# bgmanuel99/Super-Resolution-Images-for-3D-Printing-Defect-Detection

Hardware: AMD Instinct MI355X
Metric: 4x-SR MPix/s on 512x512 LR batch (higher is better)
Workload: dtype bf16

## Files before the change

super-resolution-images-for-3d-printing-defect-detection_amd/csrc/dense_fused.hip:

```cpp
#include <stdlib.h>
#include <string.h>

#include <type_traits>

#include "conv_common.h"

namespace {

struct ChainParams {
    const char* in; int in_nch;
    char* out; int out_nch;
    const char* so; int so_nch;
    const char* w;
    const float* bias;
    const char* zero;
    int B, H;
    int rows_per_wg; unsigned magic;
    float alpha, xscale, oscale;
    int dbg_flags;
    unsigned long long* dbg;
};

__device__ __forceinline__ f32x4 mma16(bf16x8 a, bf16x8 b, f32x4 c) { return __builtin_amdgcn_mfma_f32_16x16x32_bf16(a, b, c, 0, 0, 0); }

constexpr int ROWB = 3072;
constexpr int NSTG = 11;
constexpr int STGB = NSTG * ROWB;
constexpr int WINR = 10;
constexpr int ZERO_PAGE_BYTES = sr_ctx::ZERO_PAGE_BYTES;

template <int NB0, int NB1, int MODE> struct ChainLds {
    static constexpr int WSLOT = (NB0 + NB1) * 3 * 1024;
    static constexpr int NSB = MODE == 0 ? 3 : 2;
    static constexpr int NWS = MODE == 0 ? 2 : 3;
    static constexpr int BYTES = NSB * STGB + WINR * ROWB + NWS * WSLOT + (NB0 + NB1) * 16 * 4;
};

typedef unsigned u32x2 __attribute__((ext_vector_type(2)));
typedef unsigned u32x4 __attribute__((ext_vector_type(4)));
#define CHAIN_STAMP(k) do { if (STAMP && blockIdx.x < 64 && G < 64 && (wave == 0 || wave == 5 || wave == 8 || wave == 11) && lane == 0)                \
        p.dbg[(((size_t)blockIdx.x * 4 + (wave == 0 ? 0 : wave == 5 ? 1 : wave == 8 ? 2 : 3)) * 64 + G) * 4 + (k)] = __builtin_amdgcn_s_memtime(); } while (0)

template <int N, class F> __device__ __forceinline__ void static_for(F&& f) {
    if constexpr (N > 0) {
        static_for<N - 1>(f);
        f(std::integral_constant<int, N - 1>{});
    }
}

template <int N> __device__ __forceinline__ void wait_imm() {
    static_assert(N >= 0 && N < 64, "vmcnt is a 6-bit counter");
    asm volatile("s_waitcnt vmcnt(%0)" ::"n"(N) : "memory");
}

template <int EXT, int NB0, int NB1, int MODE, int LW> struct LoaderPlan {
    static constexpr int NBT = NB0 + NB1, EXTG = 3 * EXT, NGR = 3 * (EXT + 1);
    static constexpr int RT_E = MODE == 1 ? 2 : 3;
    static constexpr int RT_R = 2;
    static constexpr int nrows(int kx) { return kx == 0 ? 2 : kx == 1 ? (LW < 3 ? 1 : 0) : 0; }
    static constexpr int nst_at(int i) {
        i = (i % NGR + NGR) % NGR;
        return i < EXTG ? 3 * nrows(i % 3) : 0;
    }
    static constexpr int nwdma(int iw) {
        const bool ext = iw < EXTG;
        const int nw = ext ? NBT * 3 : NB1 * 3, rt = ext ? RT_E : RT_R;
        int n = 0;
        for (int t = 0; t < (nw + 3) / 4; ++t)
            if (LW + 4 * t < nw && t >= rt) ++n;
        return n;
    }
};

constexpr bool kDirectStores = true;
constexpr int NCOMP = 8, NLOAD = 4;

template <int EXT, int NB0, int NB1, int MODE, bool HAS_O, bool STAMP, bool SEAM = false>
__global__ void __launch_bounds__((NCOMP + NLOAD) * 64, (NCOMP + NLOAD + 3) / 4) chain2_kernel(ChainParams p) {
    using L = ChainLds<NB0, NB1, MODE>;
    constexpr int NBT = NB0 + NB1, WSLOT = L::WSLOT;
    constexpr int NGR = 3 * (EXT + 1);
    constexpr int EXTG = 3 * EXT;
    constexpr int NTHR = (NCOMP + NLOAD) * 64;
    extern __shared__ __attribute__((aligned(16))) char smem[];
    char* const stg = smem;
    constexpr int NSB = L::NSB;
    char* const win = smem + NSB * STGB;
    char* const wr = win + WINR * ROWB;
    constexpr int NWS = L::NWS;
    float* const lbias = reinterpret_cast<float*>(wr + NWS * WSLOT);

    const int tid = threadIdx.x, lane = tid & 63, px = lane & 15, q = lane >> 4;
    const int wave = __builtin_amdgcn_readfirstlane(tid >> 6);
    const int H = p.H, Hp1 = H + 1;
    const int T = p.B * Hp1;
    const int R0 = blockIdx.x * p.rows_per_wg, R1 = min(T, R0 + p.rows_per_wg);
    if (R0 >= R1) return;
    const int Rs = R0 - 1;
    const int N = R1 - Rs + 1;
    const int nsteps = (N + 1 + 7) >> 3;

    for (int u = tid; u < WINR * ROWB / 16; u += NTHR) *reinterpret_cast<f32x4*>(win + u * 16) = f32x4{0.f, 0.f, 0.f, 0.f};
    if (tid < NBT * 16) lbias[tid] = p.bias[tid];
    asm volatile("s_waitcnt lgkmcnt(0)" ::: "memory");
    __builtin_amdgcn_s_barrier();

    auto row_of = [&](int g, int& img, int& y) -> bool {
        const int gg = Rs + g;
        if (gg < 0 || gg >= T) return false;
        img = (int)__umulhi((unsigned)gg, p.magic);
        y = gg - img * Hp1;
        return y < H;
    };
    auto own = [&](int g) { return Rs + g >= R0 && Rs + g < R1; };
    int G = 0;
    auto dma = [&](const char* src, char* dst) {
        __builtin_amdgcn_global_load_lds((const __attribute__((address_space(1))) void*)src, (__attribute__((address_space(3))) void*)dst, 16, 0, 0);
    };
    if (wave >= NCOMP) {
        const int lwr = wave - NCOMP;
        const int lsrc = 64 * (lane >> 2) + 16 * ((lane & 3) ^ (2 * ((lane >> 4) & 1)));
        auto loader = [&](auto LWc) {
            constexpr int LW = decltype(LWc)::value;
            auto row_base = [&](int s2, int j) -> const char* {
                int img, y;
                const bool real = row_of(8 * s2 - 2 + j, img, y);
                return real ? p.in + ((int64_t)img * H + y) * p.in_nch * ROWB : p.zero;
            };
            using Plan = LoaderPlan<EXT, NB0, NB1, MODE, LW>;
            const char* rb_cur[3];
            const char* rb_nxt[3];
            auto bases_of = [&](int s2, const char* (&rb)[3]) {
                rb[0] = row_base(s2, LW);
                rb[1] = row_base(s2, LW + 4);
                rb[2] = row_base(s2, 8 + (LW < 3 ? LW : 2));
            };
            auto stage_row = [&](auto Jc, const char* rb, int c1, char* sdst) {
                constexpr int j = decltype(Jc)::value;
                const char* src = rb + c1 * ROWB + lsrc;
                char* dst = sdst + j * ROWB;
                const auto gs = (const __attribute__((address_space(1))) void*)src;
                const auto ld = (__attribute__((address_space(3))) void*)dst;
                if constexpr (j < 8) {
                    __builtin_amdgcn_global_load_lds(gs, ld, 16, 0, 2);
                    __builtin_amdgcn_global_load_lds(gs, ld, 16, 1024, 2);
                    __builtin_amdgcn_global_load_lds(gs, ld, 16, 2048, 2);
                } else {
                    __builtin_amdgcn_global_load_lds(gs, ld, 16, 0, 0);
                    __builtin_amdgcn_global_load_lds(gs, ld, 16, 1024, 0);
                    __builtin_amdgcn_global_load_lds(gs, ld, 16, 2048, 0);
                }
            };
            auto stage_rows = [&](auto KXc, const char* (&rb)[3], int c1, char* sdst) {
                constexpr int kx = decltype(KXc)::value;
                if constexpr (kx == 0) {
                    stage_row(std::integral_constant<int, LW>{}, rb[0], c1, sdst);
                    stage_row(std::integral_constant<int, LW + 4>{}, rb[1], c1, sdst);
                } else if constexpr (kx == 1 && LW < 3) {
                    stage_row(std::integral_constant<int, 8 + (LW < 3 ? LW : 0)>{}, rb[2], c1, sdst);
                }
            };
            constexpr int RT_E = Plan::RT_E, RT_R = Plan::RT_R;
            u32x4 wre[EXTG][RT_E], wrr[3][RT_R];
            auto wsrc_of = [&](int iw) { return p.w + (iw < EXTG ? iw * WSLOT : EXTG * WSLOT + (iw - EXTG) * (NB1 * 3 * 1024)); };
#pragma unroll
            for (int iw = 0; iw < EXTG; ++iw)
#pragma unroll
                for (int t = 0; t < RT_E; ++t)
                    if (LW + 4 * t < NBT * 3) wre[iw][t] = *reinterpret_cast<const u32x4*>(wsrc_of(iw) + (LW + 4 * t) * 1024 + lane * 16);
#pragma unroll
            for (int r = 0; r < 3; ++r)
#pragma unroll
                for (int t = 0; t < RT_R; ++t)
                    if (LW + 4 * t < NB1 * 3) wrr[r][t] = *reinterpret_cast<const u32x4*>(wsrc_of(EXTG + r) + (LW + 4 * t) * 1024 + lane * 16);
            auto put_weights = [&](auto IW, int Gw) {
                constexpr int iw = decltype(IW)::value;
                constexpr bool ext = iw < EXTG;
                constexpr int nw = ext ? NBT * 3 : NB1 * 3, rt = ext ? RT_E : RT_R;
                const char* wq = p.w;
                asm volatile("" : "+s"(wq));
                const char* wsrc = wq + (ext ? iw * WSLOT : EXTG * WSLOT + (iw - EXTG) * (NB1 * 3 * 1024)) + lane * 16;
                char* wdst = wr + (Gw % NWS) * WSLOT;
#pragma unroll
                for (int t = 0; t < (nw + 3) / 4; ++t) {
                    const int k = LW + 4 * t;
                    if (k < nw) {
                        if (t < rt) {
                            if constexpr (ext) *reinterpret_cast<u32x4*>(wdst + k * 1024 + lane * 16) = wre[ext ? iw : 0][t < RT_E ? t : 0];
                            else *reinterpret_cast<u32x4*>(wdst + k * 1024 + lane * 16) = wrr[ext ? 0 : iw - EXTG][t < RT_R ? t : 0];
                        } else {
                            dma(wsrc + k * 1024, wdst + k * 1024);
                        }
                    }
                }
            };
            constexpr int WL = NWS - 1;
            constexpr int SL = NSB - 1;
            static_assert(MODE == 1 || (RT_E * NLOAD >= NBT * 3 && RT_R * NLOAD >= NB1 * 3), "growth pairs: every weight piece is resident (no weight DMA in the counted waits)");
            static_assert(SL <= EXT, "rows run at most one step ahead");
            static_for<WL>([&](auto I) { put_weights(I, decltype(I)::value); });
            bases_of(0, rb_cur);
            bases_of(1, rb_nxt);
            static_for<SL>([&](auto C0) {
                constexpr int c0 = decltype(C0)::value;
                stage_rows(std::integral_constant<int, 0>{}, rb_cur, c0, stg + c0 * STGB);
                stage_rows(std::integral_constant<int, 1>{}, rb_cur, c0, stg + c0 * STGB);
            });
            int nch = 0;
            for (int s = 0; s < nsteps; ++s) {
                static_for<NGR>([&](auto I) {
                    constexpr int i = decltype(I)::value;
                    CHAIN_STAMP(0);
                    if (G == 0) asm volatile("s_waitcnt vmcnt(0)" ::: "memory");
                    asm volatile("s_waitcnt lgkmcnt(0)" ::: "memory");
                    __builtin_amdgcn_s_barrier();
                    CHAIN_STAMP(1);
                    constexpr int i2 = (i + WL) % NGR;
                    put_weights(std::integral_constant<int, i2>{}, G + WL);
                    if constexpr (i < EXTG) {
                        constexpr int c = i / 3, kx = i - 3 * c;
                        constexpr int c1 = (c + SL) % EXT;
                        constexpr bool next_step = c + SL >= EXT;
                        char* sdst = stg + ((nch + SL) % NSB) * STGB;
                        stage_rows(std::integral_constant<int, kx>{}, next_step ? rb_nxt : rb_cur, c1, sdst);
                        if (kx == 2) ++nch;
                    }
                    CHAIN_STAMP(2);
                    if constexpr (MODE == 0) {
                        wait_imm<Plan::nst_at(i) + Plan::nst_at(i - 1) + Plan::nst_at(i - 2)>();
                    } else {
                        constexpr bool third = i < EXTG && i % 3 == 2;
                        wait_imm<Plan::nwdma(i2) + Plan::nst_at(i) + (third ? 0 : Plan::nst_at(i - 1))>();
                    }
                    CHAIN_STAMP(3);
                    ++G;
                });
                rb_cur[0] = rb_nxt[0]; rb_cur[1] = rb_nxt[1]; rb_cur[2] = rb_nxt[2];
                bases_of(s + 2, rb_nxt);
            }
            asm volatile("s_waitcnt vmcnt(0)" ::: "memory");
        };
        if (lwr == 0) loader(std::integral_constant<int, 0>{});
        else if (lwr == 1) loader(std::integral_constant<int, 1>{});
        else if (lwr == 2) loader(std::integral_constant<int, 2>{});
        else loader(std::integral_constant<int, 3>{});
        return;
    }

    int offk[3];
#pragma unroll
    for (int kx = 0; kx < 3; ++kx) {
        const int c = px + kx - 1;
        offk[kx] = 64 * c + 16 * (q ^ (2 * ((c >> 2) & 1)));
    }
    const bool edge_l = px == 0, edge_r = px == 15;
    const int off_l = edge_l ? offk[1] : offk[0];
    const int off_r = edge_r ? offk[1] : offk[2];
    const bool seam_l = SEAM && px == 8, seam_r = SEAM && px == 7;

    f32x4 a0[NB0][3], a1[NB1][3];

    auto transpose_offsets = [&](int& t_a, int& t_line) {
        int l = lane;
        asm volatile("" : "+v"(l));
        const int px_ = l & 15, q_ = l >> 4;
        t_a = px_ * 64 + 16 * ((q_ >> 1) ^ ((px_ >> 1) & 3)) + (q_ & 1) * 8;
        t_line = (l >> 2) * 64 + 16 * ((l & 3) ^ ((l >> 3) & 3));
    };

    auto xfold = [&](int h, float scale) {
        const bf16_t xs_b = (bf16_t)scale;
        int j0 = 16 * h + px - 8 * q;
        asm volatile("" : "+v"(j0));
        bf16x8 f;
#pragma unroll
        for (int j = 0; j < 8; ++j) f[j] = j == j0 ? xs_b : (bf16_t)0.f;
        return f;
    };
    constexpr int WDEPTH = 3, NWREG = WDEPTH + 1;
    struct ExtStage { int d, layer, n, frag, first; };
    auto ext_stage = [](int k) constexpr -> ExtStage {
        int i = 0;
        for (int d = 0; d < 4; ++d) {
            bool first = true;
            if (d >= 1)
                for (int n = 0; n < NB0; ++n, ++i, first = false)
                    if (i == k) return ExtStage{d, 0, n, (d - 1) * NB0 + n, first};
            if (d <= 2)
                for (int n = 0; n < NB1; ++n, ++i, first = false)
                    if (i == k) return ExtStage{d, 1, n, 3 * NB0 + d * NB1 + n, first};
        }
        return ExtStage{-1, 0, 0, 0, 0};
    };
    constexpr int NEXTST = 3 * (NB0 + NB1);
    auto ext_granule = [&](auto KXc, auto FOLDc, const char* sb, const char* ws) {
        constexpr int KX = decltype(KXc)::value;
        constexpr int FOLD = KX == 1 ? decltype(FOLDc)::value : -1;
        const char* rb = sb + wave * ROWB;
        auto load_row = [&](int d, bf16x8 (&x)[3]) {
#pragma unroll
            for (int cg = 0; cg < 3; ++cg) {
                const int off = (KX == 0 && cg == 0) ? off_l : (KX == 2 && cg == 2) ? off_r : offk[KX];
                x[cg] = *reinterpret_cast<const bf16x8*>(rb + d * ROWB + cg * 1024 + off);
                if ((KX == 0 && cg == 0 && edge_l) || (KX == 2 && cg == 2 && edge_r)) x[cg] = bf16x8{};
                if (SEAM && cg == 1 && ((KX == 0 && seam_l) || (KX == 2 && seam_r))) x[cg] = bf16x8{};
            }
        };
        auto ldw = [&](int frag) { return *reinterpret_cast<const bf16x8*>(ws + frag * 1024 + lane * 16); };
        bf16x8 xr[2][3], wq[NWREG];
        load_row(0, xr[0]);
        static_for<WDEPTH>([&](auto K) { wq[decltype(K)::value] = ldw(ext_stage(decltype(K)::value).frag); });
        static_for<NEXTST>([&](auto K) {
            constexpr int k = decltype(K)::value;
            constexpr ExtStage st = ext_stage(k);
            if constexpr (st.first && st.d < 3) load_row(st.d + 1, xr[(st.d + 1) & 1]);
            if constexpr (k + WDEPTH < NEXTST) wq[(k + WDEPTH) % NWREG] = ldw(ext_stage(k + WDEPTH).frag);
#pragma unroll
            for (int cg = 0; cg < 3; ++cg) {
                if constexpr (st.layer == 0) a0[st.n][cg] = mma16(wq[k % NWREG], xr[st.d & 1][cg], a0[st.n][cg]);
                else a1[st.n][cg] = mma16(wq[k % NWREG], xr[st.d & 1][cg], a1[st.n][cg]);
            }
            if constexpr (FOLD >= 0 && st.d == 1 && st.layer == 1 && st.n == NB1 - 1) {
#pragma unroll
                for (int h = 0; h < 2; ++h) {
                    const bf16x8 f = xfold(h, p.xscale);
#pragma unroll
                    for (int cg = 0; cg < 3; ++cg) a1[2 * FOLD + h][cg] = mma16(f, xr[1][cg], a1[2 * FOLD + h][cg]);
                }
            }
            __builtin_amdgcn_sched_barrier(0);
        });
    };
    constexpr int NRINGST = 3 * NB1;
    auto ring_granule = [&](auto KXc, int s, const char* ws) {
        constexpr int KX = decltype(KXc)::value;
        auto load_row = [&](int ky, bf16x8 (&x)[3]) {
            const char* rb = win + ((8 * s + wave - 2 + ky + 2 * WINR) % WINR) * ROWB;
#pragma unroll
            for (int cg = 0; cg < 3; ++cg) {
                const int off = (KX == 0 && cg == 0) ? off_l : (KX == 2 && cg == 2) ? off_r : offk[KX];
                x[cg] = *reinterpret_cast<const bf16x8*>(rb + cg * 1024 + off);
                if ((KX == 0 && cg == 0 && edge_l) || (KX == 2 && cg == 2 && edge_r)) x[cg] = bf16x8{};
                if (SEAM && cg == 1 && ((KX == 0 && seam_l) || (KX == 2 && seam_r))) x[cg] = bf16x8{};
            }
        };
        auto ldw = [&](int frag) { return *reinterpret_cast<const bf16x8*>(ws + frag * 1024 + lane * 16); };
        bf16x8 xr[2][3], wq[NWREG];
        load_row(0, xr[0]);
        static_for<WDEPTH>([&](auto K) { wq[decltype(K)::value] = ldw(decltype(K)::value); });
        static_for<NRINGST>([&](auto K) {
            constexpr int k = decltype(K)::value;
            constexpr int ky = k / NB1, n = k % NB1;
            if constexpr (n == 0 && ky < 2) load_row(ky + 1, xr[(ky + 1) & 1]);
            if constexpr (k + WDEPTH < NRINGST) wq[(k + WDEPTH) % NWREG] = ldw(k + WDEPTH);
#pragma unroll
            for (int cg = 0; cg < 3; ++cg) a1[n][cg] = mma16(wq[k % NWREG], xr[ky & 1][cg], a1[n][cg]);
            __builtin_amdgcn_sched_barrier(0);
        });
    };
    auto sync = [&]() {
        asm volatile("s_waitcnt lgkmcnt(0)" ::: "memory");
        __builtin_amdgcn_s_barrier();
    };

    int nch = 0;
    auto chunk = [&](auto FOLDc, int& Gr) {
        const char* sb = stg + (nch % NSB) * STGB;
#pragma unroll
        for (int kx = 0; kx < 3; ++kx, ++Gr) {
            CHAIN_STAMP(0);
            sync();
            CHAIN_STAMP(1);
            CHAIN_STAMP(2);
            const char* ws = wr + (Gr % NWS) * WSLOT;
            if (STAMP && (p.dbg_flags & 2)) {  }
            else if (kx == 0) ext_granule(std::integral_constant<int, 0>{}, FOLDc, sb, ws);
            else if (kx == 1) ext_granule(std::integral_constant<int, 1>{}, FOLDc, sb, ws);
            else ext_granule(std::integral_constant<int, 2>{}, FOLDc, sb, ws);
            CHAIN_STAMP(3);
        }
        ++nch;
    };
    for (int s = 0; s < nsteps; ++s) {
#pragma unroll
        for (int n = 0; n < NB0; ++n) {
            const f32x4 b = *reinterpret_cast<const f32x4*>(lbias + n * 16 + 4 * q);
#pragma unroll
            for (int cg = 0; cg < 3; ++cg) a0[n][cg] = b;
        }
#pragma unroll
        for (int n = 0; n < NB1; ++n) {
            const f32x4 b = *reinterpret_cast<const f32x4*>(lbias + (NB0 + n) * 16 + 4 * q);
#pragma unroll
            for (int cg = 0; cg < 3; ++cg) a1[n][cg] = b;
        }
        if constexpr (MODE == 1) {
            static_assert(MODE == 0 || EXT >= 2, "the tail's skip spans chunks 0 and 1");
            chunk(std::integral_constant<int, 0>{}, G);
            chunk(std::integral_constant<int, 1>{}, G);
#pragma nounroll
            for (int c = 2; c < EXT; ++c) chunk(std::integral_constant<int, -1>{}, G);
        } else {
#pragma nounroll
            for (int c = 0; c < EXT; ++c) chunk(std::integral_constant<int, -1>{}, G);
        }
        {
            const int g0 = 8 * s + wave;
            int img, y;
            const bool real = row_of(g0, img, y);
            char* wrow = win + (g0 % WINR) * ROWB;
            char* grow = real && own(g0) && MODE == 0 ? const_cast<char*>(p.in) + (((int64_t)img * H + y) * p.in_nch + EXT) * ROWB : nullptr;
#pragma unroll
            for (int cg = 0; cg < 3; ++cg) {
                f32x4 v[NB0];
                bf16x4 ob[NB0];
#pragma unroll
                for (int n = 0; n < NB0; ++n) {
#pragma unroll
                    for (int e = 0; e < 4; ++e) v[n][e] = real ? fmaxf(a0[n][cg][e], 0.f) : 0.f;
                    const bf16x4 o = {(bf16_t)v[n][0], (bf16_t)v[n][1], (bf16_t)v[n][2], (bf16_t)v[n][3]};
                    ob[n] = o;
                    const int slice = n * 2 + (q >> 1);
                    *reinterpret_cast<bf16x4*>(wrow + cg * 1024 + 64 * px + 16 * (slice ^ (2 * ((px >> 2) & 1))) + (q & 1) * 8) = o;
                }
                if constexpr (MODE == 0 && NB0 == 2 && kDirectStores) {
                    if (grow) {
                        const u32x2 au = __builtin_bit_cast(u32x2, ob[0]), cu = __builtin_bit_cast(u32x2, ob[NB0 - 1]);
                        const auto s0 = __builtin_amdgcn_permlane16_swap(au[0], cu[0], false, false);
                        const auto s1 = __builtin_amdgcn_permlane16_swap(au[1], cu[1], false, false);
                        const u32x4 ov = {(unsigned)s0[0], (unsigned)s1[0], (unsigned)s0[1], (unsigned)s1[1]};
                        __builtin_nontemporal_store(ov, reinterpret_cast<u32x4*>(grow + cg * 1024 + 64 * px + 2 * ((q & 1) * 16 + 4 * (q & ~1))));
                    }
                }
            }
            if (MODE == 0 && grow && !(NB0 == 2 && kDirectStores)) {
                static_assert(MODE == 1 || NB0 == 2, "growth convs have 32 output channels");
                asm volatile("" ::: "memory");
#pragma unroll
                for (int cg = 0; cg < 3; ++cg) {
                    const u32x4 v = *reinterpret_cast<const u32x4*>(wrow + cg * 1024 + (lane >> 2) * 64 + 16 * ((lane & 3) ^ (2 * ((lane >> 4) & 1))));
                    __builtin_nontemporal_store(v, reinterpret_cast<u32x4*>(grow + cg * 1024 + lane * 16));
                }
            }
        }
        char* const tb = stg + ((nch + NSB - 1) % NSB) * STGB + wave * 4096;
        const char* sob = nullptr;
        if (MODE == 1 && HAS_O) {
            int img, y;
            if (row_of(8 * s + wave - 1, img, y) && own(8 * s + wave - 1)) sob = p.so + ((int64_t)img * H + y) * p.so_nch * ROWB;
        }
        auto so_fetch = [&](int cg) {
            if (MODE == 1 && HAS_O && sob) {
                int l = lane;
                asm volatile("" : "+v"(l));
                const int ls = 64 * (l >> 2) + 16 * ((l & 3) ^ (2 * ((l >> 4) & 1)));
                dma(sob + cg * 1024 + ls, tb);
                dma(sob + ROWB + cg * 1024 + ls, tb + 1024);
            }
        };
#pragma unroll
        for (int kx = 0; kx < 3; ++kx, ++G) {
            CHAIN_STAMP(0);
            sync();
            CHAIN_STAMP(1);
            so_fetch(kx);
            CHAIN_STAMP(2);
            const char* ws = wr + (G % NWS) * WSLOT;
            if (kx == 0) ring_granule(std::integral_constant<int, 0>{}, s, ws);
            else if (kx == 1) ring_granule(std::integral_constant<int, 1>{}, s, ws);
            else ring_granule(std::integral_constant<int, 2>{}, s, ws);
            if (MODE == 1 && HAS_O && sob) {
                asm volatile("s_waitcnt vmcnt(0)" ::: "memory");
                int l = lane;
                asm volatile("" : "+v"(l));
                const int pxl = l & 15, ql = l >> 4;
                const int offc = 64 * pxl + 16 * (ql ^ (2 * ((pxl >> 2) & 1)));
#pragma unroll
                for (int c2 = 0; c2 < 2; ++c2) {
                    const bf16x8 xo = *reinterpret_cast<const bf16x8*>(tb + c2 * 1024 + offc);
#pragma unroll
                    for (int h = 0; h < 2; ++h) a1[2 * c2 + h][kx] = mma16(xfold(h, p.oscale), xo, a1[2 * c2 + h][kx]);
                }
            }
            CHAIN_STAMP(3);
        }
        {
            int img, y;
            const bool real = row_of(8 * s + wave - 1, img, y) && own(8 * s + wave - 1);
            if (real && !(STAMP && (p.dbg_flags & 1))) {
                const int64_t rowi = (int64_t)img * H + y;
                char* const grow = MODE == 0 ? const_cast<char*>(p.in) + (rowi * p.in_nch + EXT + 1) * ROWB : p.out + rowi * p.out_nch * ROWB;
                const float alpha = p.alpha;
                int t_a, t_line;
                transpose_offsets(t_a, t_line);
                if constexpr (MODE == 0 && NB1 == 2 && kDirectStores) {
#pragma unroll
                    for (int cg = 0; cg < 3; ++cg) {
                        bf16x4 ob[2];
#pragma unroll
                        for (int n = 0; n < 2; ++n)
                            ob[n] = bf16x4{(bf16_t)fmaxf(a1[n][cg][0], 0.f), (bf16_t)fmaxf(a1[n][cg][1], 0.f), (bf16_t)fmaxf(a1[n][cg][2], 0.f), (bf16_t)fmaxf(a1[n][cg][3], 0.f)};
                        const u32x2 au = __builtin_bit_cast(u32x2, ob[0]), cu = __builtin_bit_cast(u32x2, ob[1]);
                        const auto s0 = __builtin_amdgcn_permlane16_swap(au[0], cu[0], false, false);
                        const auto s1 = __builtin_amdgcn_permlane16_swap(au[1], cu[1], false, false);
                        const u32x4 ov = {(unsigned)s0[0], (unsigned)s1[0], (unsigned)s0[1], (unsigned)s1[1]};
                        __builtin_nontemporal_store(ov, reinterpret_cast<u32x4*>(grow + cg * 1024 + 64 * px + 2 * ((q & 1) * 16 + 4 * (q & ~1))));
                    }
                } else
#pragma unroll
                for (int cg = 0; cg < 3; ++cg)
#pragma unroll
                    for (int h = 0; h < NB1 / 2; ++h) {
                        char* const slot = tb + ((2 * cg + h) & 3) * 1024;
#pragma unroll
                        for (int u = 0; u < 2; ++u) {
                            const int n = 2 * h + u;
                            f32x4 v;
#pragma unroll
                            for (int e = 0; e < 4; ++e) v[e] = MODE == 0 ? fmaxf(a1[n][cg][e], 0.f) : alpha * a1[n][cg][e];
                            *reinterpret_cast<bf16x4*>(slot + (t_a ^ (32 * u))) = bf16x4{(bf16_t)v[0], (bf16_t)v[1], (bf16_t)v[2], (bf16_t)v[3]};
                        }
                        asm volatile("" ::: "memory");
                        const u32x4 line = *reinterpret_cast<const u32x4*>(slot + t_line);
                        __builtin_nontemporal_store(line, reinterpret_cast<u32x4*>(grow + h * ROWB + cg * 1024 + lane * 16));
                    }
            }
        }
    }
}

struct Conv1Params {
    const char* in; int in_nch;
    const char* w;
    const float* bias;
    const char* zero;
    int B, H;
    int rows_per_wg; unsigned magic;
};

constexpr int C1_NSTG = 10;
constexpr int C1_STGB = C1_NSTG * ROWB;
constexpr int C1_NSB = 4;
constexpr int C1_WBYTES = 2 * 9 * 2 * 1024;
constexpr int C1_LDS = C1_NSB * C1_STGB + C1_WBYTES + 32 * 4;
static_assert(C1_LDS <= 160 * 1024, "LDS budget");

template <bool SEAM>
__global__ void __launch_bounds__((NCOMP + NLOAD) * 64, (NCOMP + NLOAD + 3) / 4) conv1_stream_kernel(Conv1Params p) {
    extern __shared__ __attribute__((aligned(16))) char smem[];
    char* const stg = smem;
    char* const lw = smem + C1_NSB * C1_STGB;
    float* const lbias = reinterpret_cast<float*>(lw + C1_WBYTES);
    constexpr int NTHR = (NCOMP + NLOAD) * 64;
    const int tid = threadIdx.x, lane = tid & 63, px = lane & 15, q = lane >> 4;
    const int wave = __builtin_amdgcn_readfirstlane(tid >> 6);
    const int H = p.H, Hp1 = H + 1;
    const int T = p.B * Hp1;
    const int R0 = blockIdx.x * p.rows_per_wg, R1 = min(T, R0 + p.rows_per_wg);
    if (R0 >= R1) return;
    const int nsteps = (R1 - R0 + 7) >> 3;
    const int nchunks = 2 * nsteps;

    for (int u = tid; u < C1_WBYTES / 16; u += NTHR) *reinterpret_cast<f32x4*>(lw + u * 16) = *reinterpret_cast<const f32x4*>(p.w + u * 16);
    if (tid < 32) lbias[tid] = p.bias[tid];

    auto row_of = [&](int g, int& img, int& y) -> bool {
        const int gg = R0 + g;
        if (gg < 0 || gg >= T) return false;
        img = (int)__umulhi((unsigned)gg, p.magic);
        y = gg - img * Hp1;
        return y < H;
    };
    if (wave >= NCOMP) {
        const int lwr = wave - NCOMP;
        const int lsrc = 64 * (lane >> 2) + 16 * ((lane & 3) ^ (2 * ((lane >> 4) & 1)));
        auto loader = [&](auto LWc) {
            constexpr int LW = decltype(LWc)::value;
            constexpr int NROWS = LW < 2 ? 3 : 2, NP = 3 * NROWS;
            auto stage_unit = [&](int k) {
                const int s2 = k >> 1, c = k & 1;
                char* const sdst = stg + (k % C1_NSB) * C1_STGB;
                static_for<NROWS>([&](auto Jc) {
                    constexpr int j = decltype(Jc)::value == 0 ? LW : decltype(Jc)::value == 1 ? LW + 4 : 8 + LW;
                    int img, y;
                    const bool real = k < nchunks && row_of(8 * s2 - 1 + j, img, y);
                    const char* src = (real ? p.in + (((int64_t)img * H + y) * p.in_nch + c) * ROWB : p.zero) + lsrc;
                    const auto gs = (const __attribute__((address_space(1))) void*)src;
                    const auto ld = (__attribute__((address_space(3))) void*)(sdst + j * ROWB);
                    __builtin_amdgcn_global_load_lds(gs, ld, 16, 0, 0);
                    __builtin_amdgcn_global_load_lds(gs, ld, 16, 1024, 0);
                    __builtin_amdgcn_global_load_lds(gs, ld, 16, 2048, 0);
                });
            };
            stage_unit(0); stage_unit(1); stage_unit(2);
            for (int k = 0; k < nchunks; ++k) {
                if (k == 0) wait_imm<2 * NP>();
                __builtin_amdgcn_s_barrier();
                stage_unit(k + 3);
                wait_imm<2 * NP>();
            }
            asm volatile("s_waitcnt vmcnt(0)" ::: "memory");
        };
        asm volatile("s_waitcnt vmcnt(0) lgkmcnt(0)" ::: "memory");
        if (lwr == 0) loader(std::integral_constant<int, 0>{});
        else if (lwr == 1) loader(std::integral_constant<int, 1>{});
        else if (lwr == 2) loader(std::integral_constant<int, 2>{});
        else loader(std::integral_constant<int, 3>{});
        return;
    }
    asm volatile("s_waitcnt vmcnt(0) lgkmcnt(0)" ::: "memory");
    int offk[3];
#pragma unroll
    for (int kx = 0; kx < 3; ++kx) {
        const int c = px + kx - 1;
        offk[kx] = 64 * c + 16 * (q ^ (2 * ((c >> 2) & 1)));
    }
    const bool edge_l = px == 0, edge_r = px == 15;
    const int off_l = edge_l ? offk[1] : offk[0];
    const int off_r = edge_r ? offk[1] : offk[2];
    typedef unsigned u32x2c __attribute__((ext_vector_type(2)));
    for (int s = 0; s < nsteps; ++s) {
        f32x4 acc[2][3];
#pragma unroll
        for (int c = 0; c < 2; ++c) {
            const int k = 2 * s + c;
            asm volatile("s_waitcnt lgkmcnt(0)" ::: "memory");
            __builtin_amdgcn_s_barrier();
            if (c == 0) {
#pragma unroll
                for (int n = 0; n < 2; ++n) {
                    const f32x4 b = *reinterpret_cast<const f32x4*>(lbias + n * 16 + 4 * q);
#pragma unroll
                    for (int cg = 0; cg < 3; ++cg) acc[n][cg] = b;
                }
            }
            const char* const sb = stg + (k % C1_NSB) * C1_STGB + wave * ROWB;
#pragma unroll
            for (int kx = 0; kx < 3; ++kx) {
                bf16x8 wf[3][2];
#pragma unroll
                for (int ky = 0; ky < 3; ++ky)
#pragma unroll
                    for (int n = 0; n < 2; ++n) wf[ky][n] = *reinterpret_cast<const bf16x8*>(lw + (((c * 9) + ky * 3 + kx) * 2 + n) * 1024 + lane * 16);
#pragma unroll
                for (int ky = 0; ky < 3; ++ky) {
#pragma unroll
                    for (int cg = 0; cg < 3; ++cg) {
                        const int off = (kx == 0 && cg == 0) ? off_l : (kx == 2 && cg == 2) ? off_r : offk[kx];
                        bf16x8 x = *reinterpret_cast<const bf16x8*>(sb + ky * ROWB + cg * 1024 + off);
                        if ((kx == 0 && cg == 0 && edge_l) || (kx == 2 && cg == 2 && edge_r)) x = bf16x8{};
                        if (SEAM && cg == 1 && ((kx == 0 && px == 8) || (kx == 2 && px == 7))) x = bf16x8{};
#pragma unroll
                        for (int n = 0; n < 2; ++n) acc[n][cg] = mma16(wf[ky][n], x, acc[n][cg]);
                    }
                }
            }
        }
        int img, y;
        const int g = 8 * s + wave;
        if (g < R1 - R0 && row_of(g, img, y)) {
            char* const grow = const_cast<char*>(p.in) + (((int64_t)img * H + y) * p.in_nch + 2) * ROWB;
            const int lane_b = 64 * px + 2 * ((q & 1) * 16 + 4 * (q & ~1));
#pragma unroll
            for (int cg = 0; cg < 3; ++cg) {
                bf16x4 o[2];
#pragma unroll
                for (int n = 0; n < 2; ++n)
                    o[n] = bf16x4{(bf16_t)fmaxf(acc[n][cg][0], 0.f), (bf16_t)fmaxf(acc[n][cg][1], 0.f), (bf16_t)fmaxf(acc[n][cg][2], 0.f), (bf16_t)fmaxf(acc[n][cg][3], 0.f)};
                const u32x2c au = __builtin_bit_cast(u32x2c, o[0]), cu = __builtin_bit_cast(u32x2c, o[1]);
                const auto s0 = __builtin_amdgcn_permlane16_swap(au[0], cu[0], false, false);
                const auto s1 = __builtin_amdgcn_permlane16_swap(au[1], cu[1], false, false);
                const u32x4 ov = {(unsigned)s0[0], (unsigned)s1[0], (unsigned)s0[1], (unsigned)s1[1]};
                __builtin_nontemporal_store(ov, reinterpret_cast<u32x4*>(grow + cg * 1024 + lane_b));
            }
        }
    }
}

template <int EXT, int NB0, int NB1, int MODE>
int launch_chain(sr_ctx* ctx, const ChainParams& p, bool has_o, int nwg, bool seam, hipStream_t st) {
    constexpr int lds = ChainLds<NB0, NB1, MODE>::BYTES;
    static_assert(lds <= 160 * 1024, "LDS budget");
    if (seam) {
        if (has_o) {
            auto k = chain2_kernel<EXT, NB0, NB1, MODE, true, false, true>;
            if (int rc = ctx->ensure_dyn_lds(reinterpret_cast<const void*>(k), lds)) return rc;
            hipLaunchKernelGGL(k, dim3(nwg), dim3((NCOMP + NLOAD) * 64), lds, st, p);
        } else {
            auto k = chain2_kernel<EXT, NB0, NB1, MODE, false, false, true>;
            if (int rc = ctx->ensure_dyn_lds(reinterpret_cast<const void*>(k), lds)) return rc;
            hipLaunchKernelGGL(k, dim3(nwg), dim3((NCOMP + NLOAD) * 64), lds, st, p);
        }
    } else if (p.dbg) {
        auto k = chain2_kernel<EXT, NB0, NB1, MODE, MODE == 1, true>;
        if (int rc = ctx->ensure_dyn_lds(reinterpret_cast<const void*>(k), lds)) return rc;
        ChainParams q = p;
        if (MODE == 1 && !has_o) { q.so = p.in; q.so_nch = p.in_nch; q.oscale = 0.f; }
        hipLaunchKernelGGL(k, dim3(nwg), dim3((NCOMP + NLOAD) * 64), lds, st, q);
    } else if (has_o) {
        auto k = chain2_kernel<EXT, NB0, NB1, MODE, true, false>;
        if (int rc = ctx->ensure_dyn_lds(reinterpret_cast<const void*>(k), lds)) return rc;
        hipLaunchKernelGGL(k, dim3(nwg), dim3((NCOMP + NLOAD) * 64), lds, st, p);
    } else {
        auto k = chain2_kernel<EXT, NB0, NB1, MODE, false, false>;
        if (int rc = ctx->ensure_dyn_lds(reinterpret_cast<const void*>(k), lds)) return rc;
        hipLaunchKernelGGL(k, dim3(nwg), dim3((NCOMP + NLOAD) * 64), lds, st, p);
    }
    SR_HIP(ctx, hipGetLastError());
    return SR_OK;
}

}

int chain_pack_weights(sr_ctx* ctx, const float* wa, const float* ba, const float* wb, const float* bb, int ext, int nb0, int nb1, ChainWeights* out) {
    const int cin_a = 32 * ext, cin_b = 32 * (ext + 1), cout_a = 16 * nb0, cout_b = 16 * nb1;
    const size_t nfrag = (size_t)3 * ext * 3 * (nb0 + nb1) + (size_t)3 * 3 * nb1;
    std::vector<uint16_t> host(nfrag * 512);
    size_t idx = 0;
    auto frag = [&](const float* w, int cin, int cout, int c, int ky, int kx, int blk) {
        for (int l = 0; l < 64; ++l)
            for (int j = 0; j < 8; ++j)
                host[idx++] = f32_to_bf16_host(w[((size_t)(ky * 3 + kx) * cin + 32 * c + 8 * (l >> 4) + j) * cout + 16 * blk + (l & 15)]);
    };
    for (int c = 0; c < ext; ++c)
        for (int kx = 0; kx < 3; ++kx) {
            for (int ky = 0; ky < 3; ++ky) for (int n = 0; n < nb0; ++n) frag(wa, cin_a, cout_a, c, ky, kx, n);
            for (int ky = 0; ky < 3; ++ky) for (int n = 0; n < nb1; ++n) frag(wb, cin_b, cout_b, c, ky, kx, n);
        }
    for (int kx = 0; kx < 3; ++kx)
        for (int ky = 0; ky < 3; ++ky) for (int n = 0; n < nb1; ++n) frag(wb, cin_b, cout_b, ext, ky, kx, n);
    ChainWeights cw;
    cw.ext = ext; cw.nb0 = nb0; cw.nb1 = nb1;
    cw.bytes = host.size() * 2;
    std::vector<float> hb(cout_a + cout_b, 0.f);
    if (ba) for (int i = 0; i < cout_a; ++i) hb[i] = ba[i];
    if (bb) for (int i = 0; i < cout_b; ++i) hb[cout_a + i] = bb[i];
    if (int rc = weights_upload(ctx, host.data(), cw.bytes, hb.data(), (int)hb.size(), (int)hb.size(), &cw.w, &cw.bias)) return rc;
    *out = cw;
    return SR_OK;
}

bool conv1_stream_supported(const ConvWeights& w, const TensorView& in, int W) {
    return w.w != nullptr && w.rows && w.dtype == SR_DTYPE_BF16 && w.KS == 3 && w.Cin == 64 && w.Cout == 32 && w.NT == 2 && w.nchunks == 2 && W == 48 && in.blk &&
           in.coff == 0 && in.cs % 32 == 0 && in.cs >= 96;
}

int conv1_stream_launch(sr_ctx* ctx, const ConvWeights& w, TensorView in, int B, int H, int W, hipStream_t st, bool seam) {
    if (!conv1_stream_supported(w, in, W)) return ctx->fail(SR_ERR_INVALID, "streaming conv1: needs a 64 -> 32 bf16 3x3 conv on a 48-pixel-wide row-blocked buffer");
    if (B <= 0 || H <= 0) return ctx->fail(SR_ERR_INVALID, "streaming conv1: empty tensor");
    if (!ctx->zero_page) return ctx->fail(SR_ERR_STATE, "context has no zero page");
    int ncu = ctx->cu_count();
    if (ctx->chain_max_wgs > 0 && ctx->chain_max_wgs < ncu) ncu = ctx->chain_max_wgs;
    Conv1Params p;
    p.in = static_cast<const char*>(in.p); p.in_nch = (int)(in.cs / 32);
    p.w = static_cast<const char*>(w.w); p.bias = w.bias; p.zero = static_cast<const char*>(ctx->zero_page);
    p.B = B; p.H = H;
    const int64_t T = (int64_t)B * (H + 1);
    if ((T + 16) * (int64_t)(H + 1) * (H + 1) >= (1ll << 32)) return ctx->fail(SR_ERR_INVALID, "streaming conv1: stream too long");
    const int nwg_target = (int)std::max<int64_t>(1, std::min<int64_t>(ncu, (T + 15) / 16));
    p.rows_per_wg = (int)((T + nwg_target - 1) / nwg_target);
    const int nwg = (int)((T + p.rows_per_wg - 1) / p.rows_per_wg);
    p.magic = (unsigned)(((1ull << 32) + (unsigned)H) / (unsigned)(H + 1));
    int rec = -1;
    if (ctx->prof) {
        const double px = (double)B * H * W;
        rec = ctx->prof_open("dense_conv1_stream<bf16,64->32>", 2.0 * px * 9.0 * 64 * 32, px * 2.0 * (64 + 32), st);
    }
    auto k = seam ? conv1_stream_kernel<true> : conv1_stream_kernel<false>;
    if (int rc = ctx->ensure_dyn_lds(reinterpret_cast<const void*>(k), C1_LDS)) return rc;
    hipLaunchKernelGGL(k, dim3(nwg), dim3((NCOMP + NLOAD) * 64), C1_LDS, st, p);
    ctx->prof_close(rec, st);
    SR_HIP(ctx, hipGetLastError());
    return SR_OK;
}

bool chain_supported(const ChainWeights& w, const TensorView& in, int W) {
    return w.w != nullptr && W == 48 && in.blk && in.coff == 0 && in.cs % 32 == 0 && in.cs >= 32 * (w.ext + (w.nb1 == 4 ? 1 : 2));
}

int chain_launch(sr_ctx* ctx, const ChainWeights& w, TensorView in, int B, int H, int W, TensorView out, TensorView skip_o, float alpha,
                 float beta_x, float beta_o, hipStream_t st, bool seam) {
    if (!chain_supported(w, in, W)) return ctx->fail(SR_ERR_INVALID, "fused dense-block pair: needs W == 48 and a row-blocked source buffer");
    if (B <= 0 || H <= 0) return ctx->fail(SR_ERR_INVALID, "fused dense-block pair: empty tensor");
    const bool tail = w.nb1 == 4;
    if (tail && (!out.p || !out.blk || out.coff != 0 || out.cs % 32 != 0 || alpha == 0.f)) return ctx->fail(SR_ERR_INVALID, "fused dense-block tail: bad destination view");
    if (skip_o.p && (!skip_o.blk || skip_o.coff != 0 || skip_o.cs % 32 != 0)) return ctx->fail(SR_ERR_INVALID, "fused dense-block tail: bad skip view");
    static_assert(ZERO_PAGE_BYTES >= 6 * ROWB, "zero page covers every chunk offset");
    if (!ctx->zero_page) return ctx->fail(SR_ERR_STATE, "context has no zero page");
    int ncu = ctx->num_cus;
    if (ncu <= 0) {
        hipDeviceProp_t prop;
        SR_HIP(ctx, hipGetDeviceProperties(&prop, ctx->device));
        ncu = ctx->num_cus = prop.multiProcessorCount > 0 ? prop.multiProcessorCount : 256;
    }
    if (ctx->chain_max_wgs > 0 && ctx->chain_max_wgs < ncu) ncu = ctx->chain_max_wgs;
    ChainParams p;
    p.in = static_cast<const char*>(in.p); p.in_nch = (int)(in.cs / 32);
    p.out = static_cast<char*>(const_cast<void*>(out.p)); p.out_nch = (int)(out.cs / 32);
    p.so = static_cast<const char*>(skip_o.p); p.so_nch = (int)(skip_o.cs / 32);
    p.w = static_cast<const char*>(w.w); p.bias = w.bias; p.zero = static_cast<const char*>(ctx->zero_page);
    p.B = B; p.H = H;
    const int64_t T = (int64_t)B * (H + 1);
    if ((T + 16) * (int64_t)(H + 1) * (H + 1) >= (1ll << 32)) return ctx->fail(SR_ERR_INVALID, "fused dense-block pair: stream too long");
    const int nwg_target = (int)std::max<int64_t>(1, std::min<int64_t>(ncu, (T + 23) / 24));
    p.rows_per_wg = (int)((T + nwg_target - 1) / nwg_target);
    const int nwg = (int)((T + p.rows_per_wg - 1) / p.rows_per_wg);
    p.magic = (unsigned)(((1ull << 32) + (unsigned)H) / (unsigned)(H + 1));
    p.alpha = alpha; p.xscale = tail ? beta_x / alpha : 0.f; p.oscale = tail && skip_o.p ? beta_o / alpha : 0.f;
    for (float sc : {p.xscale, p.oscale}) {
        uint32_t u = (uint32_t)f32_to_bf16_host(sc) << 16;
        float back;
        memcpy(&back, &u, 4);
        if (back != sc) return ctx->fail(SR_ERR_INVALID, "fused dense-block tail: beta / alpha is not exactly representable in bf16");
    }
    p.dbg = ctx->chain_stamp_buf;
    { const char* f = getenv("SR355_CHAIN_DBG_FLAGS"); p.dbg_flags = f ? atoi(f) : 0; }
    if (p.dbg && ctx->chain_stamp_skip >= 0 && ctx->chain_stamp_skip-- != 0) p.dbg = nullptr;
    if (p.dbg && ctx->chain_stamp_skip == -1 && getenv("SR355_CHAIN_STAMP_SKIP")) ctx->chain_stamp_buf = nullptr;
    int rec = -1;
    if (ctx->prof) {
        const double px = (double)B * H * W;
        const double cin_a = 32.0 * w.ext, cin_b = 32.0 * (w.ext + 1), ca = 16.0 * w.nb0, cb = 16.0 * w.nb1;
        double bytes = px * 2.0 * (cin_a + (tail ? cb : ca + cb));
        if (tail && skip_o.p) bytes += px * 2.0 * 64.0;
        rec = ctx->prof_open(tail ? "dense_tail_fused<bf16,conv4+conv5>" : "dense_pair_fused<bf16>", 2.0 * px * 9.0 * (cin_a * ca + cin_b * cb), bytes, st);
    }
    int rc;
    const bool has_o = skip_o.p != nullptr;
    if (tail && w.ext == 5 && w.nb0 == 2) rc = launch_chain<5, 2, 4, 1>(ctx, p, has_o, nwg, seam, st);
    else if (!tail && w.ext == 2 && w.nb0 == 2 && w.nb1 == 2) rc = launch_chain<2, 2, 2, 0>(ctx, p, false, nwg, seam, st);
    else if (!tail && w.ext == 3 && w.nb0 == 2 && w.nb1 == 2) rc = launch_chain<3, 2, 2, 0>(ctx, p, false, nwg, seam, st);
    else rc = ctx->fail(SR_ERR_INVALID, "fused dense-block pair: shape not instantiated");
    ctx->prof_close(rec, st);
    return rc;
}
```

Baseline: 111.3.

## Prefetch outer-skip rows directly into registers ahead of the ring granules

The outer-skip rows used in the tail MMA were previously loaded by DMA into LDS staging per kx and waited on with a full vmcnt(0). They are now loaded straight into registers with global loads. The first column group is issued during the last external chunk and the other two before the ring loop, with graded vmcnt waits per kx. This is meant to hide global latency and drop the LDS round trip and the full drains. In exchange it holds six extra bf16x8 registers live, reads from a zero buffer for rows that are not real, and needs EXT >= 3.

After: 111.6 (median of 6 runs). No clear change (+0.3%).

```diff
diff --git a/super-resolution-images-for-3d-printing-defect-detection_amd/csrc/dense_fused.hip b/super-resolution-images-for-3d-printing-defect-detection_amd/csrc/dense_fused.hip
--- a/super-resolution-images-for-3d-printing-defect-detection_amd/csrc/dense_fused.hip
+++ b/super-resolution-images-for-3d-printing-defect-detection_amd/csrc/dense_fused.hip
@@ -363,14 +363,31 @@
         __builtin_amdgcn_s_barrier();
     };
 
+    bf16x8 xo[3][2];
+    auto so_issue = [&](int s, auto CGc) {
+        if constexpr (MODE == 1 && HAS_O) {
+            constexpr int cg = decltype(CGc)::value;
+            int img, y;
+            const int g1 = 8 * s + wave - 1;
+            const char* sob = row_of(g1, img, y) && own(g1) ? p.so + ((int64_t)img * H + y) * p.so_nch * ROWB : p.zero;
+            int l = lane;
+            asm volatile("" : "+v"(l));
+            const char* src = sob + (unsigned)(cg * 1024 + 64 * (l & 15) + 16 * (l >> 4));
+#pragma unroll
+            for (int c2 = 0; c2 < 2; ++c2) xo[cg][c2] = *reinterpret_cast<const bf16x8*>(src + c2 * ROWB);
+        }
+    };
     int nch = 0;
-    auto chunk = [&](auto FOLDc, int& Gr) {
+    auto chunk = [&](auto FOLDc, auto SOc, int s, int& Gr) {
         const char* sb = stg + (nch % NSB) * STGB;
 #pragma unroll
         for (int kx = 0; kx < 3; ++kx, ++Gr) {
             CHAIN_STAMP(0);
             sync();
             CHAIN_STAMP(1);
+            if constexpr (decltype(SOc)::value) {
+                if (kx == 2) so_issue(s, std::integral_constant<int, 0>{});
+            }
             CHAIN_STAMP(2);
             const char* ws = wr + (Gr % NWS) * WSLOT;
             if (STAMP && (p.dbg_flags & 2)) {  }
@@ -396,13 +413,15 @@
         }
         if constexpr (MODE == 1) {
             static_assert(MODE == 0 || EXT >= 2, "the tail's skip spans chunks 0 and 1");
-            chunk(std::integral_constant<int, 0>{}, G);
-            chunk(std::integral_constant<int, 1>{}, G);
+            static_assert(!HAS_O || EXT >= 3, "the last external chunk carries no x skip");
+            chunk(std::integral_constant<int, 0>{}, std::false_type{}, s, G);
+            chunk(std::integral_constant<int, 1>{}, std::false_type{}, s, G);
 #pragma nounroll
-            for (int c = 2; c < EXT; ++c) chunk(std::integral_constant<int, -1>{}, G);
+            for (int c = 2; c < EXT - (HAS_O ? 1 : 0); ++c) chunk(std::integral_constant<int, -1>{}, std::false_type{}, s, G);
+            if constexpr (HAS_O) chunk(std::integral_constant<int, -1>{}, std::true_type{}, s, G);
         } else {
 #pragma nounroll
-            for (int c = 0; c < EXT; ++c) chunk(std::integral_constant<int, -1>{}, G);
+            for (int c = 0; c < EXT; ++c) chunk(std::integral_constant<int, -1>{}, std::false_type{}, s, G);
         }
         {
             const int g0 = 8 * s + wave;
@@ -444,43 +463,26 @@
             }
         }
         char* const tb = stg + ((nch + NSB - 1) % NSB) * STGB + wave * 4096;
-        const char* sob = nullptr;
-        if (MODE == 1 && HAS_O) {
-            int img, y;
-            if (row_of(8 * s + wave - 1, img, y) && own(8 * s + wave - 1)) sob = p.so + ((int64_t)img * H + y) * p.so_nch * ROWB;
-        }
-        auto so_fetch = [&](int cg) {
-            if (MODE == 1 && HAS_O && sob) {
-                int l = lane;
-                asm volatile("" : "+v"(l));
-                const int ls = 64 * (l >> 2) + 16 * ((l & 3) ^ (2 * ((l >> 4) & 1)));
-                dma(sob + cg * 1024 + ls, tb);
-                dma(sob + ROWB + cg * 1024 + ls, tb + 1024);
-            }
-        };
+        so_issue(s, std::integral_constant<int, 1>{});
+        so_issue(s, std::integral_constant<int, 2>{});
 #pragma unroll
         for (int kx = 0; kx < 3; ++kx, ++G) {
             CHAIN_STAMP(0);
             sync();
             CHAIN_STAMP(1);
-            so_fetch(kx);
             CHAIN_STAMP(2);
             const char* ws = wr + (G % NWS) * WSLOT;
             if (kx == 0) ring_granule(std::integral_constant<int, 0>{}, s, ws);
             else if (kx == 1) ring_granule(std::integral_constant<int, 1>{}, s, ws);
             else ring_granule(std::integral_constant<int, 2>{}, s, ws);
-            if (MODE == 1 && HAS_O && sob) {
-                asm volatile("s_waitcnt vmcnt(0)" ::: "memory");
-                int l = lane;
-                asm volatile("" : "+v"(l));
-                const int pxl = l & 15, ql = l >> 4;
-                const int offc = 64 * pxl + 16 * (ql ^ (2 * ((pxl >> 2) & 1)));
-#pragma unroll
-                for (int c2 = 0; c2 < 2; ++c2) {
-                    const bf16x8 xo = *reinterpret_cast<const bf16x8*>(tb + c2 * 1024 + offc);
-#pragma unroll
-                    for (int h = 0; h < 2; ++h) a1[2 * c2 + h][kx] = mma16(xfold(h, p.oscale), xo, a1[2 * c2 + h][kx]);
-                }
+            if constexpr (MODE == 1 && HAS_O) {
+                if (kx == 0) wait_imm<4>();
+                else if (kx == 1) wait_imm<2>();
+                else wait_imm<0>();
+#pragma unroll
+                for (int c2 = 0; c2 < 2; ++c2)
+#pragma unroll
+                    for (int h = 0; h < 2; ++h) a1[2 * c2 + h][kx] = mma16(xfold(h, p.oscale), xo[kx][c2], a1[2 * c2 + h][kx]);
             }
             CHAIN_STAMP(3);
         }
```
